# HumaticsLAB/SEAM-Match-RCNN

Hardware: NVIDIA B200
Metric: pair_scores_per_sec (higher is better)
Workload: dtype f32 (fp16-operand tcgen05 pass nominates candidates, every result re-scored in f32)

## Files before the change

seam-match-rcnn_b200/csrc/score_exact.cuh:

```cuda
#pragma once
#include <type_traits>
#include <climits>
#include <cstdint>
#include <cuda_fp16.h>
#include "exchange.cuh"
#include "fold.cuh"
#include "score_tc.cuh"
#include "sm100_ptx.cuh"
#include "warp_sort.cuh"

namespace seam {
namespace exact {

constexpr float FP16_MAX = 65504.f;
constexpr float EPS_COEFF = 9.9e-4f;
constexpr float TAG_REL_ERR = 8e-6f;

__device__ __forceinline__ float softmax1(float l0, float l1) {
  const float m = fmaxf(l0, l1);
  const float e0 = expf(l0 - m), e1 = expf(l1 - m);
  return e1 / (e0 + e1);
}

struct Slice {
  float4 lo, hi;
};
__device__ __forceinline__ Slice load_slice(const float* row, int lane) {
  Slice s;
  s.lo = *reinterpret_cast<const float4*>(row + 4 * lane);
  s.hi = *reinterpret_cast<const float4*>(row + 128 + 4 * lane);
  return s;
}
__device__ __forceinline__ float4 widen4(uint2 v) {
  const float2 a = __half22float2(*reinterpret_cast<const __half2*>(&v.x));
  const float2 b = __half22float2(*reinterpret_cast<const __half2*>(&v.y));
  return make_float4(a.x, a.y, b.x, b.y);
}
__device__ __forceinline__ Slice load_slice(const __half* row, int lane) {
  Slice s;
  s.lo = widen4(*reinterpret_cast<const uint2*>(row + 4 * lane));
  s.hi = widen4(*reinterpret_cast<const uint2*>(row + 128 + 4 * lane));
  return s;
}
typedef unsigned long long u64;
__device__ __forceinline__ u64 pk2(float lo, float hi) {
  u64 r;
  asm("mov.b64 %0, {%1, %2};" : "=l"(r) : "f"(lo), "f"(hi));
  return r;
}
__device__ __forceinline__ float sum2(u64 v) {
  float lo, hi;
  asm("mov.b64 {%0, %1}, %2;" : "=f"(lo), "=f"(hi) : "l"(v));
  return lo + hi;
}
__device__ __forceinline__ void sqdiff_dot2(const Slice& q, const Slice& g, const Slice& w0, const Slice& w1,
                                            float& p0, float& p1) {
  u64 a0, a1, d, s;
#define SEAM_TERM2(F, X, Y, FIRST)                                                                   \
  asm("sub.rn.f32x2 %0, %1, %2;" : "=l"(d) : "l"(pk2(q.F.X, q.F.Y)), "l"(pk2(g.F.X, g.F.Y)));      \
  asm("mul.rn.f32x2 %0, %1, %1;" : "=l"(s) : "l"(d));                                               \
  if (FIRST) {                                                                                       \
    asm("mul.rn.f32x2 %0, %1, %2;" : "=l"(a0) : "l"(pk2(w0.F.X, w0.F.Y)), "l"(s));                  \
    asm("mul.rn.f32x2 %0, %1, %2;" : "=l"(a1) : "l"(pk2(w1.F.X, w1.F.Y)), "l"(s));                  \
  } else {                                                                                           \
    asm("fma.rn.f32x2 %0, %1, %2, %0;" : "+l"(a0) : "l"(pk2(w0.F.X, w0.F.Y)), "l"(s));              \
    asm("fma.rn.f32x2 %0, %1, %2, %0;" : "+l"(a1) : "l"(pk2(w1.F.X, w1.F.Y)), "l"(s));              \
  }
  SEAM_TERM2(lo, x, y, true) SEAM_TERM2(lo, z, w, false) SEAM_TERM2(hi, x, y, false) SEAM_TERM2(hi, z, w, false)
#undef SEAM_TERM2
  p0 = sum2(a0);
  p1 = sum2(a1);
}
template <typename Row>
__device__ __forceinline__ void pair_logits(const Slice& q, const Row* grow, const Slice& w0, const Slice& w1,
                                            float b0, float b1, int lane, float& l0, float& l1) {
  const Slice g = load_slice(grow, lane);
  float p0, p1;
  sqdiff_dot2(q, g, w0, w1, p0, p1);
  l0 = ptx::warp_sum_b(p0) + b0;
  l1 = ptx::warp_sum_b(p1) + b1;
}

template <typename Row>
__global__ void __launch_bounds__(256) prep_gallery_kernel(const Row* __restrict__ g, int G,
                                                           const float* __restrict__ fold, __half* __restrict__ g16,
                                                           float* __restrict__ cg, float* __restrict__ gstat) {
  const int warp = threadIdx.x >> 5, lane = threadIdx.x & 31;
  const int j = blockIdx.x * 8 + warp;
  if (j >= G) return;
  const Slice x = load_slice(g + (size_t)j * 256, lane);
  const Slice dw = load_slice(fold + Fold::DW, lane);
  const float xs[8] = {x.lo.x, x.lo.y, x.lo.z, x.lo.w, x.hi.x, x.hi.y, x.hi.z, x.hi.w};
  const float ds[8] = {dw.lo.x, dw.lo.y, dw.lo.z, dw.lo.w, dw.hi.x, dw.hi.y, dw.hi.z, dw.hi.w};
  float c = 0.f, n2 = 0.f, amax = 0.f;
  __half h[8];
#pragma unroll
  for (int e = 0; e < 8; ++e) {
    c = fmaf(ds[e], xs[e] * xs[e], c);
    n2 = fmaf(xs[e], xs[e], n2);
    amax = fmaxf(amax, fabsf(xs[e]));
    h[e] = __float2half_rn(xs[e]);
  }
  if constexpr (std::is_same<Row, float>::value) {
    __half* dst = g16 + (size_t)j * 256;
    *reinterpret_cast<uint2*>(dst + 4 * lane) = *reinterpret_cast<const uint2*>(&h[0]);
    *reinterpret_cast<uint2*>(dst + 128 + 4 * lane) = *reinterpret_cast<const uint2*>(&h[4]);
  }
  c = ptx::warp_sum(c);
  n2 = ptx::warp_sum(n2);
  amax = ptx::warp_max(amax);
  if (lane == 0) {
    cg[j] = c;
    atomicMax(reinterpret_cast<unsigned int*>(gstat), __float_as_uint(sqrtf(n2)));
    if (!(amax < FP16_MAX)) atomicMax(reinterpret_cast<unsigned int*>(gstat + 1), __float_as_uint(1.f));
  }
}

__global__ void __launch_bounds__(256) prep_queries_kernel(const float* q, int Q,
                                                           const float* __restrict__ fold, __half* __restrict__ a16,
                                                           float* __restrict__ rq, float* __restrict__ anorm,
                                                           uint32_t* __restrict__ thr_global,
                                                           uint32_t* __restrict__ rowflag,
                                                           int32_t* __restrict__ counters,
                                                           int32_t* __restrict__ xdone, const int x_on,
                                                           const xchg::Exchange xc) {
  const int warp = threadIdx.x >> 5, lane = threadIdx.x & 31;
  const int i = blockIdx.x * 8 + warp;
  if (x_on) {
    const uint32_t step = xchg::current_step(xc);
    xchg::wait_all(xc, xchg::KIND_Q, step);
    q = xc.q_all[xc.rank] + (size_t)(step & 1u) * xc.Q * 256;
  }
  if (blockIdx.x == 0 && threadIdx.x == 0) {
    counters[0] = 0;
    counters[1] = 0;
  }
  if (i >= Q) return;
  const Slice x = load_slice(q + (size_t)i * 256, lane);
  const Slice dw = load_slice(fold + Fold::DW, lane);
  const float xs[8] = {x.lo.x, x.lo.y, x.lo.z, x.lo.w, x.hi.x, x.hi.y, x.hi.z, x.hi.w};
  const float ds[8] = {dw.lo.x, dw.lo.y, dw.lo.z, dw.lo.w, dw.hi.x, dw.hi.y, dw.hi.z, dw.hi.w};
  float r = 0.f, n2 = 0.f, amax = 0.f;
  __half h[8];
#pragma unroll
  for (int e = 0; e < 8; ++e) {
    const float a = -2.f * ds[e] * xs[e];
    r = fmaf(ds[e], xs[e] * xs[e], r);
    n2 = fmaf(a, a, n2);
    amax = fmaxf(amax, fabsf(a));
    h[e] = __float2half_rn(a);
  }
  __half* dst = a16 + (size_t)i * 256;
  *reinterpret_cast<uint2*>(dst + 4 * lane) = *reinterpret_cast<const uint2*>(&h[0]);
  *reinterpret_cast<uint2*>(dst + 128 + 4 * lane) = *reinterpret_cast<const uint2*>(&h[4]);
  r = ptx::warp_sum(r);
  n2 = ptx::warp_sum(n2);
  amax = ptx::warp_max(amax);
  if (lane == 0) {
    rq[i] = r;
    anorm[i] = sqrtf(n2);
    thr_global[i] = ptx::float_to_ordered(-INFINITY);
    rowflag[i] = 0;
    if (xdone) xdone[i] = 0;
    if (!(amax < FP16_MAX)) atomicExch(counters + 1, 1);
  }
}

struct RescoreParams {
  const float* q;
  const void* g;
  const float* fold;
  const uint2* rowbuf;
  const uint32_t* rowcnt;
  const uint32_t* rowflag;
  const uint32_t* thr_global;
  const float* gmax;
  const float* rq;
  const float* anorm;
  const float* gstat;
  int Q, G, nlists, CAP, k, index_offset;
  float* out_score;
  float* out_margin;
  int32_t* out_idx;
  int32_t* counters;
  int32_t* fallback_rows;
  int x_on;
  xchg::Exchange x;
  score::TilePlan plan;
};

struct TopkDest {
  float* score;
  float* margin;
  int32_t* idx;
};
__device__ __forceinline__ TopkDest topk_dest(int x_on, const xchg::Exchange& x, uint32_t step, int qi, int k,
                                              float* out_score, float* out_margin, int32_t* out_idx) {
  TopkDest d;
  if (!x_on) {
    const size_t o = (size_t)qi * k;
    d.score = out_score + o;
    d.margin = out_margin + o;
    d.idx = out_idx + o;
  } else {
    const int ow = xchg::owner_of(x, qi);
    const size_t o = ((((size_t)(step & 1u) * x.world + x.rank) * x.own_max) + (size_t)(qi - x.q_lo[ow])) * k;
    d.score = nullptr;
    d.margin = x.list_margin[ow] + o;
    d.idx = x.list_idx[ow] + o;
  }
  return d;
}

constexpr int RS_SUBL = 4;
constexpr int RESCORE_WBUF = 160;

__device__ __forceinline__ void rescore_merge32(const uint2* wb, int begin, int end, float& cv, uint32_t& cidx,
                                                int lane) {
  float v = -INFINITY;
  uint32_t id = 0xffffffffu;
  if (begin + lane < end) {
    const uint2 e = wb[begin + lane];
    v = __uint_as_float(e.x);
    id = e.y;
  }
  const float worst = __shfl_sync(ptx::FULL_MASK, cv, 31);
  if (!(v > worst)) {
    v = -INFINITY;
    id = 0xffffffffu;
  }
  if (!__any_sync(ptx::FULL_MASK, v > -INFINITY)) return;
  wsort::sort32<false>(v, id, lane);
  if (v > cv) {
    cv = v;
    cidx = id;
  }
  wsort::merge32<true>(cv, cidx, lane);
}

template <typename Row>
__global__ void __launch_bounds__(256) rescore_kernel(const RescoreParams p) {
  __shared__ uint2 wbuf[8][RESCORE_WBUF];
  __shared__ uint4 qbuf[8][64];
  __shared__ uint32_t qcol[8][64];
  const int warp = threadIdx.x >> 5, lane = threadIdx.x & 31;
  const int qi = blockIdx.x * 8 + warp;
  if (qi >= p.Q) return;
  const uint32_t xstep = p.x_on ? xchg::current_step(p.x) : 0u;
  const float* qbase = p.x_on ? p.x.q_all[p.x.rank] + (size_t)(xstep & 1u) * p.x.Q * 256 : p.q;
  const bool overflow = p.counters[1] != 0 || p.gstat[1] != 0.f;
  bool certified = !overflow && p.rowflag[qi] == 0;
  const float tau = ptx::ordered_to_float(p.thr_global[qi]);
  const int nl_valid = min(p.nlists, 4 * score::pieces_of_row(p.plan, qi));
  float cv = -INFINITY;
  uint32_t cidx = 0xffffffffu;
  uint2* wb = wbuf[warp];
  int fill = 0;
  float cut = tau;
  bool cut_strict = false;
  float cut_lo = tau > -INFINITY ? nextafterf(tau, -INFINITY) : -INFINITY;
  {
    const int nval = nl_valid * 16;
    const float* gmp = p.gmax + (size_t)qi * p.nlists * 16;
    auto start_cut = [&](auto nk_tag) {
      constexpr int NK = decltype(nk_tag)::value;
      uint32_t key[NK];
#pragma unroll
      for (int u = 0; u < NK; ++u) {
        const int i = lane + 32 * u;
        key[u] = i < nval ? ptx::float_to_ordered(gmp[i]) : 0u;
      }
      uint32_t lmax = key[0];
#pragma unroll
      for (int j = 1; j < NK; ++j) lmax = max(lmax, key[j]);
      const uint32_t hi = __reduce_max_sync(ptx::FULL_MASK, lmax);
      const uint32_t lo = __reduce_min_sync(ptx::FULL_MASK, lmax);
      uint32_t K = lo;
      if (hi != lo) {
        const int b0 = 31 - __clz(hi ^ lo);
        K = hi & ~((2u << b0) - 1u);
        for (int b = b0; b >= 0 && b > b0 - 8; --b) {
          const uint32_t T = K | (1u << b);
          uint32_t c = 0;
#pragma unroll
          for (int j = 0; j < NK; ++j)
            asm("{\n.reg .pred p;\nsetp.ge.u32 p, %1, %2;\n@p add.u32 %0, %0, 1;\n}\n" : "+r"(c) : "r"(key[j]), "r"(T));
          if (__reduce_add_sync(ptx::FULL_MASK, c) >= 32u) K = T;
        }
      }
      const float tt = ptx::ordered_to_float(K);
      if (K != 0 && tt > cut) {
        cut = tt;
        cut_lo = nextafterf(tt, -INFINITY);
      }
    };
    if (nval <= 128) start_cut(std::integral_constant<int, 4>{});
    else if (nval <= 256) start_cut(std::integral_constant<int, 8>{});
  }
  const int capq = p.CAP / 2;
  const uint4* rowq = reinterpret_cast<const uint4*>(p.rowbuf) + (size_t)qi * p.nlists * capq;
  uint4* qb = qbuf[warp];
  uint32_t* qc = qcol[warp];
  int qfill = 0;
  auto expand = [&](int start, int count) {
    uint4 rec = make_uint4(0u, 0u, 0u, 0u);
    uint32_t col = 0;
    const bool have = lane < count;
    if (have) {
      rec = qb[start + lane];
      col = qc[start + lane];
    }
    const uint32_t wv[4] = {rec.x, rec.y, rec.z, rec.w};
#pragma unroll
    for (int el = 0; el < 4; ++el) {
      const float ev = __uint_as_float(wv[el]);
      const bool pass = have && ev > cut_lo;
      const uint32_t mask = __ballot_sync(ptx::FULL_MASK, pass);
      if (mask == 0u) continue;
      if (pass) wb[fill + __popc(mask & ((1u << lane) - 1u))] = make_uint2(wv[el], col + el);
      fill += __popc(mask);
    }
    if (fill >= 32) {
      __syncwarp();
      while (fill >= 32) {
        rescore_merge32(wb, fill - 32, fill, cv, cidx, lane);
        fill -= 32;
      }
      const float worst = __shfl_sync(ptx::FULL_MASK, cv, 31);
      if (worst > cut || (worst == cut && worst > -INFINITY)) {
        cut = worst;
        cut_strict = true;
        cut_lo = worst;
      }
    }
    __syncwarp();
  };
  for (int l0 = 0; l0 < nl_valid && certified; l0 += 32) {
    const int my_l = l0 + lane;
    uint32_t my_n = my_l < nl_valid ? p.rowcnt[(size_t)qi * p.nlists + my_l] : 0u;
    if (__any_sync(ptx::FULL_MASK, my_n > (uint32_t)capq)) {
      certified = false;
      break;
    }
    const int nl = min(32, nl_valid - l0);
    for (int j0 = 0; j0 < nl; j0 += RS_SUBL) {
      int n4[RS_SUBL];
      int nmax = 0;
#pragma unroll
      for (int u = 0; u < RS_SUBL; ++u) {
        n4[u] = (int)__shfl_sync(ptx::FULL_MASK, my_n, j0 + u);
        nmax = max(nmax, n4[u]);
      }
      const uint4* lp = rowq + (size_t)(l0 + j0) * capq + lane;
      for (int base = 0; base < nmax; base += 32) {
        uint4 e[RS_SUBL];
#pragma unroll
        for (int u = 0; u < RS_SUBL; ++u)
          e[u] = base + lane < n4[u] ? __ldcs(lp + (size_t)u * capq + base)
                                     : make_uint4(0xff800000u, 0xff800000u, 0xff800000u, 0xff800000u);
#pragma unroll
        for (int u = 0; u < RS_SUBL; ++u) {
          const float m = fmaxf(fmaxf(__uint_as_float(e[u].x), __uint_as_float(e[u].y)),
                                fmaxf(__uint_as_float(e[u].z), __uint_as_float(e[u].w)));
          const bool pass = m > cut_lo;
          const uint32_t mask = __ballot_sync(ptx::FULL_MASK, pass);
          if (mask == 0u) continue;
          if (pass) {
            const int pos = qfill + __popc(mask & ((1u << lane) - 1u));
            qb[pos] = e[u];
            qc[pos] = score::quad_first_col(e[u], l0 + j0 + u);
          }
          qfill += __popc(mask);
          if (qfill >= 32) {
            __syncwarp();
            expand(qfill - 32, 32);
            qfill -= 32;
          }
        }
      }
    }
  }
  __syncwarp();
  if (certified && qfill > 0) expand(0, qfill);
  __syncwarp();
  if (certified && fill > 0) rescore_merge32(wb, 0, fill, cv, cidx, lane);
  const bool valid = (int)cidx >= 0;
  const int n_valid = __popc(__ballot_sync(ptx::FULL_MASK, valid));
  if (n_valid < min(32, p.G)) certified = false;
  const float a_k = __shfl_sync(ptx::FULL_MASK, cv, min(p.k, 32) - 1);
  const float amax = ptx::warp_max(valid ? fabsf(cv) : 0.f);
  const float eps = EPS_COEFF * p.anorm[qi] * p.gstat[0] + 1e-5f + TAG_REL_ERR * amax;
  const float cutoff = a_k - 2.f * eps;
  const bool in_S = valid && cv >= cutoff;
  const uint32_t smask = __ballot_sync(ptx::FULL_MASK, in_S);
  if (p.G > 32 && (smask >> 31)) certified = false;
  const int ns = __popc(smask);

  const Slice qs = load_slice(qbase + (size_t)qi * 256, lane);
  const Slice w0 = load_slice(p.fold + Fold::LAST_W, lane);
  const Slice w1 = load_slice(p.fold + Fold::LAST_W + 256, lane);
  const float b0 = p.fold[Fold::CONSTS + 5], b1 = p.fold[Fold::CONSTS + 6];
  float my_l0 = 0.f, my_l1 = 0.f;
  if (certified) {
    for (int c0 = 0; c0 < ns; c0 += 4) {
      Slice gs[4];
#pragma unroll
      for (int u = 0; u < 4; ++u) {
        const int idx = __shfl_sync(ptx::FULL_MASK, (int)cidx, min(c0 + u, ns - 1));
        gs[u] = load_slice(static_cast<const Row*>(p.g) + (size_t)idx * 256, lane);
      }
      float part[8];
#pragma unroll
      for (int u = 0; u < 4; ++u) sqdiff_dot2(qs, gs[u], w0, w1, part[2 * u], part[2 * u + 1]);
      const float tot = ptx::treduce<8>(part, lane);
      const int u_mine = lane - c0;
      const float l0 = __shfl_sync(ptx::FULL_MASK, tot, (2 * u_mine) & 7) + b0;
      const float l1 = __shfl_sync(ptx::FULL_MASK, tot, (2 * u_mine + 1) & 7) + b1;
      if (u_mine >= 0 && u_mine < 4) {
        my_l0 = l0;
        my_l1 = l1;
      }
    }
  }
  float d = in_S ? my_l1 - my_l0 : -INFINITY;
  int id = in_S ? (int)cidx : INT_MAX;
  const float approx_d = cv + p.rq[qi] + p.fold[Fold::CONSTS + 4];
  const bool violated = in_S && !(fabsf(d - approx_d) <= eps + 2e-5f * (1.f + fabsf(d)));
  if (__any_sync(ptx::FULL_MASK, violated)) certified = false;
  wsort::sort32_rank2(d, id, lane);
  if (lane < p.k) {
    const TopkDest dst = topk_dest(p.x_on, p.x, xstep, qi, p.k, p.out_score, p.out_margin, p.out_idx);
    const bool ok = id != INT_MAX;
    if (dst.score) dst.score[lane] = ok ? softmax1(0.f, d) : 0.f;
    dst.margin[lane] = d;
    dst.idx[lane] = ok ? id + p.index_offset : -1;
  }
  if (!certified && lane == 0) {
    const int slot = atomicAdd(p.counters, 1);
    p.fallback_rows[slot] = qi;
  }
}

struct ExactParams {
  const float* q;
  const void* g;
  const float* fold;
  int Q, G, k, index_offset;
  const int32_t* count;
  const int32_t* rows;
  float* out_score;
  float* out_margin;
  int32_t* out_idx;
  float* part_d;
  int32_t* part_i;
  int32_t* done;
  int x_on;
  xchg::Exchange x;
};

constexpr int EXACT_MIN_SLICE = 128;

template <typename Row>
__global__ void __launch_bounds__(256) exact_topk_kernel(const ExactParams p) {
  __shared__ float sd[8][32];
  __shared__ int si[8][32];
  __shared__ int s_last;
  const int warp = threadIdx.x >> 5, lane = threadIdx.x & 31;
  const int nrows = p.count ? *p.count : p.Q;
  const uint32_t xstep = p.x_on ? xchg::current_step(p.x) : 0u;
  const float* qbase = p.x_on ? p.x.q_all[p.x.rank] + (size_t)(xstep & 1u) * p.x.Q * 256 : p.q;
  int S = 1;
  if (p.part_d && nrows > 0 && nrows < (int)gridDim.x) S = max(1, min((int)gridDim.x / nrows, p.G / EXACT_MIN_SLICE));
  const long long units = (long long)nrows * S;
  if (units == 0) {
    if (p.x_on) xchg::signal_all(p.x, xchg::KIND_L, xstep, false);
    return;
  }
  const Slice w0 = load_slice(p.fold + Fold::LAST_W, lane);
  const Slice w1 = load_slice(p.fold + Fold::LAST_W + 256, lane);
  const float b0 = p.fold[Fold::CONSTS + 5], b1 = p.fold[Fold::CONSTS + 6];
  float cd;
  int cidx;
  auto cta_merge = [&]() {
    sd[warp][lane] = cd;
    si[warp][lane] = cidx;
    __syncthreads();
    if (warp == 0) {
      float dummy = 0.f;
      for (int w = 1; w < 8; ++w) {
        const float od = sd[w][31 - lane];
        const int oi = si[w][31 - lane];
        if (wsort::ranks_before(od, oi, cd, cidx)) {
          cd = od;
          cidx = oi;
        }
        wsort::merge32_rank(cd, cidx, dummy, lane);
      }
    }
  };
  auto write_row = [&](int qi) {
    if (lane < p.k) {
      const TopkDest dst = topk_dest(p.x_on, p.x, xstep, qi, p.k, p.out_score, p.out_margin, p.out_idx);
      const bool ok = cidx != INT_MAX;
      if (dst.score) dst.score[lane] = ok ? softmax1(0.f, cd) : 0.f;
      dst.margin[lane] = cd;
      dst.idx[lane] = ok ? cidx + p.index_offset : -1;
    }
  };
  for (long long e = blockIdx.x; e < units; e += gridDim.x) {
    const int r = (int)(e / S), sl = (int)(e - (long long)r * S);
    const int qi = p.count ? p.rows[r] : r;
    const int j_lo = (int)((long long)p.G * sl / S), j_hi = (int)((long long)p.G * (sl + 1) / S);
    const Slice qs = load_slice(qbase + (size_t)qi * 256, lane);
    cd = -INFINITY;
    cidx = INT_MAX;
    for (int j0 = j_lo + 4 * warp; j0 < j_hi; j0 += 32) {
      Slice gs[4];
#pragma unroll
      for (int u = 0; u < 4; ++u) gs[u] = load_slice(static_cast<const Row*>(p.g) + (size_t)min(j0 + u, j_hi - 1) * 256, lane);
      float part[8];
#pragma unroll
      for (int u = 0; u < 4; ++u) sqdiff_dot2(qs, gs[u], w0, w1, part[2 * u], part[2 * u + 1]);
      const float tot = ptx::treduce<8>(part, lane);
#pragma unroll
      for (int u = 0; u < 4; ++u) {
        const float l0 = __shfl_sync(ptx::FULL_MASK, tot, 2 * u) + b0;
        const float l1 = __shfl_sync(ptx::FULL_MASK, tot, 2 * u + 1) + b1;
        const float d = l1 - l0;
        const int j = j0 + u;
        const float wd = __shfl_sync(ptx::FULL_MASK, cd, 31);
        const int wi = __shfl_sync(ptx::FULL_MASK, cidx, 31);
        if (j < j_hi && wsort::ranks_before(d, j, wd, wi)) {
          const int pos = __popc(__ballot_sync(ptx::FULL_MASK, wsort::ranks_before(cd, cidx, d, j)));
          const float ud = __shfl_up_sync(ptx::FULL_MASK, cd, 1);
          const int ui = __shfl_up_sync(ptx::FULL_MASK, cidx, 1);
          if (lane > pos) {
            cd = ud;
            cidx = ui;
          } else if (lane == pos) {
            cd = d;
            cidx = j;
          }
        }
      }
    }
    cta_merge();
    if (S == 1) {
      if (warp == 0) write_row(qi);
      __syncthreads();
      continue;
    }
    if (warp == 0) {
      __stcg(p.part_d + (size_t)e * 32 + lane, cd);
      __stcg(p.part_i + (size_t)e * 32 + lane, cidx);
      __threadfence();
      __syncwarp();
      if (lane == 0) s_last = atomicAdd(p.done + r, 1) == S - 1;
    }
    __syncthreads();
    if (s_last) {
      __threadfence();
      cd = -INFINITY;
      cidx = INT_MAX;
      float dummy = 0.f;
      for (int s2 = warp; s2 < S; s2 += 8) {
        const size_t o = ((size_t)r * S + s2) * 32 + (31 - lane);
        const float od = __ldcg(p.part_d + o);
        const int oi = __ldcg(p.part_i + o);
        if (wsort::ranks_before(od, oi, cd, cidx)) {
          cd = od;
          cidx = oi;
        }
        wsort::merge32_rank(cd, cidx, dummy, lane);
      }
      __syncthreads();
      cta_merge();
      if (warp == 0) {
        write_row(qi);
        if (lane == 0) p.done[r] = 0;
      }
    }
    __syncthreads();
  }
  if (p.x_on) {
    __syncthreads();
    xchg::signal_all(p.x, xchg::KIND_L, xstep, (long long)blockIdx.x < units);
  }
}

template <bool PROB>
__global__ void __launch_bounds__(256) dense_logits_kernel(const float* __restrict__ q, int Q,
                                                           const float* __restrict__ g, int G,
                                                           const float* __restrict__ fold, float* __restrict__ x5) {
  __shared__ float qs[32][129];
  __shared__ float gs[32][129];
  __shared__ float ws[2][256];
  const int t = threadIdx.x;
  const int i0 = blockIdx.y * 32, j0 = blockIdx.x * 32;
  ws[0][t] = fold[Fold::LAST_W + t];
  ws[1][t] = fold[Fold::LAST_W + 256 + t];
  const int tx = t & 31, ty = t >> 5;
  float l0[4] = {}, l1[4] = {};
  for (int kh = 0; kh < 256; kh += 128) {
    __syncthreads();
    for (int e = t; e < 32 * 128; e += 256) {
      const int r = e >> 7, c = e & 127;
      qs[r][c] = (i0 + r < Q) ? q[(size_t)(i0 + r) * 256 + kh + c] : 0.f;
      gs[r][c] = (j0 + r < G) ? g[(size_t)(j0 + r) * 256 + kh + c] : 0.f;
    }
    __syncthreads();
    for (int k = 0; k < 128; ++k) {
      const float gv = gs[tx][k];
      const float wa = ws[0][kh + k], wb = ws[1][kh + k];
#pragma unroll
      for (int u = 0; u < 4; ++u) {
        const float d = qs[ty * 4 + u][k] - gv;
        const float s = d * d;
        l0[u] = fmaf(wa, s, l0[u]);
        l1[u] = fmaf(wb, s, l1[u]);
      }
    }
  }
  const float b0 = fold[Fold::CONSTS + 5], b1 = fold[Fold::CONSTS + 6];
#pragma unroll
  for (int u = 0; u < 4; ++u) {
    const int i = i0 + ty * 4 + u, j = j0 + tx;
    if (i < Q && j < G) {
      if constexpr (PROB) {
        x5[(size_t)i * G + j] = softmax1(l0[u] + b0, l1[u] + b1);
      } else {
        float2 o = make_float2(l0[u] + b0, l1[u] + b1);
        *reinterpret_cast<float2*>(x5 + ((size_t)i * G + j) * 2) = o;
      }
    }
  }
}

struct FusedDistParams {
  const float* frames;
  const int32_t* start;
  const float* g;
  const int32_t* target;
  const float* fold;
  int P, G;
  int32_t* rank_avg;
  int32_t* rank_max;
};
constexpr int FD_ROWS = 1024, FD_FRAMES = 16;

__global__ void __launch_bounds__(256) fused_dist_rank_kernel(const FusedDistParams p) {
  __shared__ __align__(16) float fs[FD_FRAMES][256];
  __shared__ float acc_sum[FD_ROWS + 1], acc_max[FD_ROWS + 1];
  __shared__ int cnt_s[2];
  const int warp = threadIdx.x >> 5, lane = threadIdx.x & 31;
  const int prod = blockIdx.x, j0 = blockIdx.y * FD_ROWS;
  const int f0 = p.start[prod], nf = p.start[prod + 1] - f0;
  if (nf <= 0) {
    if (blockIdx.y == 0 && threadIdx.x == 0) {
      p.rank_avg[prod] = p.G;
      p.rank_max[prod] = p.G;
    }
    return;
  }
  const int rows = min(FD_ROWS, p.G - j0);
  const int tj = p.target[prod];
  for (int i = threadIdx.x; i <= FD_ROWS; i += 256) {
    acc_sum[i] = 0.f;
    acc_max[i] = -INFINITY;
  }
  if (threadIdx.x < 2) cnt_s[threadIdx.x] = 0;
  const Slice w0 = load_slice(p.fold + Fold::LAST_W, lane);
  const Slice w1 = load_slice(p.fold + Fold::LAST_W + 256, lane);
  const float b0 = p.fold[Fold::CONSTS + 5], b1 = p.fold[Fold::CONSTS + 6];
  for (int c0 = 0; c0 < nf; c0 += FD_FRAMES) {
    const int nc = min(FD_FRAMES, nf - c0);
    __syncthreads();
    for (int e = threadIdx.x; e < nc * 64; e += 256)
      reinterpret_cast<float4*>(&fs[0][0])[e] = reinterpret_cast<const float4*>(p.frames + (size_t)(f0 + c0) * 256)[e];
    __syncthreads();
    for (int r = warp; r <= rows; r += 8) {
      const int j = r < rows ? j0 + r : tj;
      const int slot = r < rows ? r : FD_ROWS;
      const Slice gs = load_slice(p.g + (size_t)j * 256, lane);
      float sum = 0.f, mx = -INFINITY;
      for (int fb = 0; fb < nc; fb += 4) {
        float part[8];
#pragma unroll
        for (int u = 0; u < 4; ++u) {
          const Slice fr = load_slice(&fs[min(fb + u, nc - 1)][0], lane);
          sqdiff_dot2(fr, gs, w0, w1, part[2 * u], part[2 * u + 1]);
        }
        const float tot = ptx::treduce<8>(part, lane);
#pragma unroll
        for (int u = 0; u < 4; ++u) {
          const float l0 = __shfl_sync(ptx::FULL_MASK, tot, 2 * u) + b0;
          const float l1 = __shfl_sync(ptx::FULL_MASK, tot, 2 * u + 1) + b1;
          if (fb + u < nc) {
            const float pr = softmax1(l0, l1);
            sum += pr;
            mx = fmaxf(mx, pr);
          }
        }
      }
      if (lane == 0) {
        acc_sum[slot] += sum;
        acc_max[slot] = fmaxf(acc_max[slot], mx);
      }
    }
  }
  __syncthreads();
  const float inv = 1.f / (float)nf;
  const float tavg = acc_sum[FD_ROWS] * inv, tmax = acc_max[FD_ROWS];
  int ca = 0, cm = 0;
  for (int i = threadIdx.x; i < rows; i += 256) {
    const int j = j0 + i;
    const float a = acc_sum[i] * inv, m = acc_max[i];
    ca += (a > tavg || (a == tavg && j < tj)) ? 1 : 0;
    cm += (m > tmax || (m == tmax && j < tj)) ? 1 : 0;
  }
  ca = __reduce_add_sync(ptx::FULL_MASK, ca);
  cm = __reduce_add_sync(ptx::FULL_MASK, cm);
  if (lane == 0) {
    atomicAdd(&cnt_s[0], ca);
    atomicAdd(&cnt_s[1], cm);
  }
  __syncthreads();
  if (threadIdx.x == 0) {
    atomicAdd(p.rank_avg + prod, cnt_s[0]);
    atomicAdd(p.rank_max + prod, cnt_s[1]);
  }
}

template <typename Row>
__global__ void __launch_bounds__(256) rank_of_target_kernel(const float* __restrict__ q, int Q,
                                                             const Row* __restrict__ g, int G,
                                                             const int32_t* __restrict__ target,
                                                             const float* __restrict__ fold,
                                                             const int32_t* __restrict__ count,
                                                             const int32_t* __restrict__ rows,
                                                             int32_t* __restrict__ out_rank,
                                                             float* __restrict__ out_margin) {
  __shared__ int cnt_s[8];
  const int warp = threadIdx.x >> 5, lane = threadIdx.x & 31;
  const Slice w0 = load_slice(fold + Fold::LAST_W, lane);
  const Slice w1 = load_slice(fold + Fold::LAST_W + 256, lane);
  const float b0 = fold[Fold::CONSTS + 5], b1 = fold[Fold::CONSTS + 6];
  const int nrows = count ? *count : Q;
  for (int e = blockIdx.x; e < nrows; e += gridDim.x) {
    const int qi = count ? rows[e] : e;
    const Slice qs = load_slice(q + (size_t)qi * 256, lane);
    const int tj = target[qi];
    float l0, l1;
    pair_logits(qs, g + (size_t)tj * 256, w0, w1, b0, b1, lane, l0, l1);
    const float dt = l1 - l0;
    int cnt = 0;
    for (int j = warp; j < G; j += 8) {
      pair_logits(qs, g + (size_t)j * 256, w0, w1, b0, b1, lane, l0, l1);
      if (wsort::ranks_before(l1 - l0, j, dt, tj)) ++cnt;
    }
    if (lane == 0) cnt_s[warp] = cnt;
    __syncthreads();
    if (threadIdx.x == 0) {
      int tot = 0;
      for (int w = 0; w < 8; ++w) tot += cnt_s[w];
      out_rank[qi] = tot;
      if (out_margin) out_margin[qi] = dt;
    }
    __syncthreads();
  }
}

template <typename Row>
__global__ void __launch_bounds__(256) rank_prep_kernel(const float* __restrict__ q, int Q, const Row* __restrict__ g,
                                                        const int32_t* __restrict__ target,
                                                        const float* __restrict__ fold, const float* __restrict__ rq,
                                                        const float* __restrict__ anorm,
                                                        const float* __restrict__ gstat, float* __restrict__ lo,
                                                        float* __restrict__ hi, float* __restrict__ dtarget,
                                                        int32_t* __restrict__ above, int nlists) {
  const int warp = threadIdx.x >> 5, lane = threadIdx.x & 31;
  const int qi = blockIdx.x * 8 + warp;
  if (qi >= Q) return;
  const Slice w0 = load_slice(fold + Fold::LAST_W, lane);
  const Slice w1 = load_slice(fold + Fold::LAST_W + 256, lane);
  const float b0 = fold[Fold::CONSTS + 5], b1 = fold[Fold::CONSTS + 6];
  const Slice qs = load_slice(q + (size_t)qi * 256, lane);
  float l0, l1;
  pair_logits(qs, g + (size_t)target[qi] * 256, w0, w1, b0, b1, lane, l0, l1);
  const float dt = l1 - l0;
  for (int l = lane; l < nlists; l += 32) above[(size_t)qi * nlists + l] = 0;
  if (lane == 0) {
    const float vstar = dt - rq[qi] - fold[Fold::CONSTS + 4];
    const float e0 = EPS_COEFF * anorm[qi] * gstat[0] + 1e-5f;
    const float E = e0 + TAG_REL_ERR * (fabsf(vstar) + e0) + 4e-6f * (1.f + fabsf(dt) + fabsf(vstar));
    lo[qi] = vstar - E;
    hi[qi] = vstar + E;
    dtarget[qi] = dt;
  }
}

struct RankResolveParams {
  const float* q;
  const void* g;
  const float* fold;
  const uint2* rowbuf;
  const uint32_t* rowcnt;
  const uint32_t* rowflag;
  const int32_t* above;
  const float* lo;
  const float* hi;
  const float* dtarget;
  const float* rq;
  const float* gstat;
  const int32_t* target;
  int Q, G, nlists, CAP;
  score::TilePlan plan;
  int32_t* out_rank;
  float* out_margin;
  int32_t* counters;
  int32_t* fallback_rows;
};
constexpr int RANK_CAND = 96;

template <typename Row>
__global__ void __launch_bounds__(256) rank_resolve_kernel(const RankResolveParams p) {
  __shared__ uint2 cand[8][RANK_CAND + 128];
  const int warp = threadIdx.x >> 5, lane = threadIdx.x & 31;
  const int qi = blockIdx.x * 8 + warp;
  if (qi >= p.Q) return;
  const bool overflow = p.counters[1] != 0 || p.gstat[1] != 0.f;
  bool ok = !overflow && p.rowflag[qi] == 0;
  const float lo = p.lo[qi], hi = p.hi[qi], dt = p.dtarget[qi];
  const int tj = p.target[qi];
  const int capq = p.CAP / 2;
  const uint4* rowq = reinterpret_cast<const uint4*>(p.rowbuf) + (size_t)qi * p.nlists * capq;
  uint2* cb = cand[warp];
  const Slice qs = load_slice(p.q + (size_t)qi * 256, lane);
  const Slice w0 = load_slice(p.fold + Fold::LAST_W, lane);
  const Slice w1 = load_slice(p.fold + Fold::LAST_W + 256, lane);
  const float b0 = p.fold[Fold::CONSTS + 5], b1 = p.fold[Fold::CONSTS + 6];
  const float eps = 0.5f * (hi - lo);
  const float shift = p.rq[qi] + p.fold[Fold::CONSTS + 4];
  int total = 0, fill = 0, exact_before = 0;
  auto decide = [&]() {
    __syncwarp();
    for (int c0 = 0; c0 < fill; c0 += 4) {
      Slice gs[4];
      uint2 ce[4];
#pragma unroll
      for (int u = 0; u < 4; ++u) {
        ce[u] = cb[min(c0 + u, fill - 1)];
        gs[u] = load_slice(static_cast<const Row*>(p.g) + (size_t)ce[u].y * 256, lane);
      }
      float part[8];
#pragma unroll
      for (int u = 0; u < 4; ++u) sqdiff_dot2(qs, gs[u], w0, w1, part[2 * u], part[2 * u + 1]);
      const float tot = ptx::treduce<8>(part, lane);
#pragma unroll
      for (int u = 0; u < 4; ++u) {
        const float l0v = __shfl_sync(ptx::FULL_MASK, tot, 2 * u) + b0;
        const float l1v = __shfl_sync(ptx::FULL_MASK, tot, 2 * u + 1) + b1;
        const float d = l1v - l0v;
        if (c0 + u < fill) {
          if (wsort::ranks_before(d, (int)ce[u].y, dt, tj)) ++exact_before;
          if (!(fabsf(d - (__uint_as_float(ce[u].x) + shift)) <= eps)) ok = false;
        }
      }
    }
    fill = 0;
    __syncwarp();
  };
  const int nl_valid = min(p.nlists, 4 * score::pieces_of_row(p.plan, qi));
  for (int l0 = 0; l0 < nl_valid && ok; l0 += 32) {
    const int my_l = l0 + lane;
    const uint32_t my_n = my_l < nl_valid ? p.rowcnt[(size_t)qi * p.nlists + my_l] : 0u;
    total += my_l < nl_valid ? p.above[(size_t)qi * p.nlists + my_l] : 0;
    if (__any_sync(ptx::FULL_MASK, my_n > (uint32_t)capq)) ok = false;
    const int nl = min(32, nl_valid - l0);
    for (int j = 0; j < nl && ok; ++j) {
      const int n = (int)__shfl_sync(ptx::FULL_MASK, my_n, j);
      const uint4* lp = rowq + (size_t)(l0 + j) * capq;
      for (int base = 0; base < n && ok; base += 32) {
        const bool have = base + lane < n;
        const uint4 rec = have ? __ldcs(lp + base + lane) : make_uint4(0u, 0u, 0u, 0u);
        const uint32_t wv[4] = {rec.x, rec.y, rec.z, rec.w};
        const uint32_t col = score::quad_first_col(rec, l0 + j);
#pragma unroll
        for (int el = 0; el < 4; ++el) {
          const float ev = __uint_as_float(wv[el]);
          const bool in_band = have && ev > lo && !(ev > hi);
          const uint32_t mask = __ballot_sync(ptx::FULL_MASK, in_band);
          if (mask == 0u) continue;
          if (in_band) cb[fill + __popc(mask & ((1u << lane) - 1u))] = make_uint2(wv[el], col + el);
          fill += __popc(mask);
        }
        if (fill >= RANK_CAND) decide();
      }
    }
  }
  total = __reduce_add_sync(ptx::FULL_MASK, total);
  if (ok && fill > 0) decide();
  if (lane == 0) {
    if (ok) {
      p.out_rank[qi] = total + exact_before;
      if (p.out_margin) p.out_margin[qi] = dt;
    } else {
      const int slot = atomicAdd(p.counters, 1);
      p.fallback_rows[slot] = qi;
    }
  }
}

__global__ void __launch_bounds__(256) merge_topk_kernel(const float* __restrict__ scores,
                                                         const float* __restrict__ margins,
                                                         const int32_t* __restrict__ idx, int N, int Q, int k,
                                                         float* __restrict__ out_score,
                                                         float* __restrict__ out_margin,
                                                         int32_t* __restrict__ out_idx) {
  const int warp = threadIdx.x >> 5, lane = threadIdx.x & 31;
  const int qi = blockIdx.x * 8 + warp;
  if (qi >= Q) return;
  float d = -INFINITY, s = 0.f;
  int id = INT_MAX;
  for (int n = 0; n < N; ++n) {
    const size_t base = ((size_t)n * Q + qi) * k;
    if (n == 0) {
      if (lane < k && idx[base + lane] >= 0) {
        d = margins[base + lane];
        s = scores ? scores[base + lane] : 0.f;
        id = idx[base + lane];
      }
    } else {
      const int e = 31 - lane;
      float od = -INFINITY, os = 0.f;
      int oi = INT_MAX;
      if (e < k && idx[base + e] >= 0) {
        od = margins[base + e];
        os = scores ? scores[base + e] : 0.f;
        oi = idx[base + e];
      }
      if (wsort::ranks_before(od, oi, d, id)) {
        d = od;
        id = oi;
        s = os;
      }
      wsort::merge32_rank(d, id, s, lane);
    }
  }
  if (lane < k) {
    const size_t o = (size_t)qi * k + lane;
    const bool ok = id != INT_MAX;
    out_score[o] = ok ? (scores ? s : softmax1(0.f, d)) : 0.f;
    out_margin[o] = ok ? d : -INFINITY;
    out_idx[o] = ok ? id : -1;
  }
}

__global__ void __launch_bounds__(256) merge_sharded_kernel(const xchg::Exchange x, float* __restrict__ out_score,
                                                            float* __restrict__ out_margin,
                                                            int32_t* __restrict__ out_idx) {
  const int warp = threadIdx.x >> 5, lane = threadIdx.x & 31;
  const uint32_t step = xchg::current_step(x);
  xchg::wait_all(x, xchg::KIND_L, step);
  const int own = x.q_lo[x.rank + 1] - x.q_lo[x.rank], k = x.k;
  const int qo = blockIdx.x * 8 + warp;
  if (qo < own) {
    const float* margins = x.list_margin[x.rank] + (size_t)(step & 1u) * x.world * x.own_max * k;
    const int32_t* idx = x.list_idx[x.rank] + (size_t)(step & 1u) * x.world * x.own_max * k;
    float d = -INFINITY, s = 0.f;
    int id = INT_MAX;
    for (int n = 0; n < x.world; ++n) {
      const size_t base = ((size_t)n * x.own_max + qo) * k;
      const int e = n == 0 ? lane : 31 - lane;
      float od = -INFINITY;
      int oi = INT_MAX;
      if (e < k) {
        const int32_t ii = __ldcg(idx + base + e);
        if (ii >= 0) {
          od = __ldcg(margins + base + e);
          oi = ii;
        }
      }
      if (n == 0) {
        d = od;
        id = oi;
      } else {
        if (wsort::ranks_before(od, oi, d, id)) {
          d = od;
          id = oi;
        }
        wsort::merge32_rank(d, id, s, lane);
      }
    }
    if (lane < k) {
      const bool ok = id != INT_MAX;
      const float sc = ok ? softmax1(0.f, d) : 0.f;
      const float dm = ok ? d : -INFINITY;
      const int ii = ok ? id : -1;
      if (x.final_score[0]) {
        const size_t o = (size_t)(x.q_lo[x.rank] + qo) * k + lane;
        if (x.final_score_mc) {
          x.final_score_mc[o] = sc;
          x.final_margin_mc[o] = dm;
          x.final_idx_mc[o] = ii;
        } else {
          for (int r = 0; r < x.world; ++r) {
            x.final_score[r][o] = sc;
            x.final_margin[r][o] = dm;
            x.final_idx[r][o] = ii;
          }
        }
      } else {
        const size_t o = (size_t)qo * k + lane;
        out_score[o] = sc;
        out_margin[o] = dm;
        out_idx[o] = ii;
      }
    }
  }
  __syncthreads();
  if (xchg::signal_all(x, xchg::KIND_F, step)) {
    if (x.final_score[0]) {
      for (int r = 0; r < x.world; ++r) {
        const uint32_t* f = x.flags[x.rank] + xchg::KIND_F * xchg::MAX_WORLD + r;
        uint64_t t0 = 0;
        while ((int32_t)(xchg::ld_acquire_sys(f) - step) < 0) {
          __nanosleep(100);
          const uint64_t now = ptx::globaltimer_ns();
          if (t0 == 0) t0 = now;
          else if (now - t0 > 10000000000ull) ptx::watchdog_trap(210u, (uint32_t)r, step);
        }
      }
    }
    *reinterpret_cast<volatile uint32_t*>(x.step) = step + 1u;
  }
}

}
}
```

seam-match-rcnn_b200/csrc/warp_sort.cuh:

```cuda
#pragma once
#include <cstdint>
#include "sm100_ptx.cuh"

namespace seam {
namespace wsort {

template <bool DESC>
__device__ __forceinline__ void cmpx(float& v, uint32_t& p, int lane, int j, int k) {
  const float ov = __shfl_xor_sync(ptx::FULL_MASK, v, j);
  const uint32_t op = __shfl_xor_sync(ptx::FULL_MASK, p, j);
  const bool keep_min = ((((lane & k) == 0) == ((lane & j) == 0)) != DESC);
  const float nv = keep_min ? fminf(v, ov) : fmaxf(v, ov);
  if (nv != v) p = op;
  v = nv;
}
template <bool DESC>
__device__ __forceinline__ void sort32(float& v, uint32_t& p, int lane) {
#pragma unroll
  for (int k = 2; k <= 32; k <<= 1)
#pragma unroll
    for (int j = k >> 1; j > 0; j >>= 1) cmpx<DESC>(v, p, lane, j, k);
}
template <bool DESC>
__device__ __forceinline__ void merge32(float& v, uint32_t& p, int lane) {
#pragma unroll
  for (int j = 16; j > 0; j >>= 1) cmpx<DESC>(v, p, lane, j, 32);
}

__device__ __forceinline__ bool ranks_before(float da, int ia, float db, int ib) {
  return da > db || (da == db && ia < ib);
}
__device__ __forceinline__ void cmpx_rank(float& d, int& i, float& s, int lane, int j, int k) {
  const float od = __shfl_xor_sync(ptx::FULL_MASK, d, j);
  const int oi = __shfl_xor_sync(ptx::FULL_MASK, i, j);
  const float os = __shfl_xor_sync(ptx::FULL_MASK, s, j);
  const bool up = (lane & k) == 0;
  const bool lower = (lane & j) == 0;
  const bool keep_better = (lower == up);
  const bool take = keep_better ? ranks_before(od, oi, d, i) : ranks_before(d, i, od, oi);
  if (take) {
    d = od;
    i = oi;
    s = os;
  }
}
__device__ __forceinline__ void cmpx_rank2(float& d, int& i, int lane, int j, int k) {
  const float od = __shfl_xor_sync(ptx::FULL_MASK, d, j);
  const int oi = __shfl_xor_sync(ptx::FULL_MASK, i, j);
  const bool up = (lane & k) == 0;
  const bool lower = (lane & j) == 0;
  const bool keep_better = (lower == up);
  const bool take = keep_better ? ranks_before(od, oi, d, i) : ranks_before(d, i, od, oi);
  if (take) {
    d = od;
    i = oi;
  }
}
__device__ __forceinline__ void sort32_rank2(float& d, int& i, int lane) {
  uint32_t hi = ptx::float_to_ordered(d), lo = ~(uint32_t)i;
#pragma unroll
  for (int k = 2; k <= 32; k <<= 1)
#pragma unroll
    for (int j = k >> 1; j > 0; j >>= 1) {
      const uint32_t ohi = __shfl_xor_sync(ptx::FULL_MASK, hi, j);
      const uint32_t olo = __shfl_xor_sync(ptx::FULL_MASK, lo, j);
      const bool keep_better = ((lane & k) == 0) == ((lane & j) == 0);
      const bool other_better = ohi > hi || (ohi == hi && olo > lo);
      if (other_better == keep_better) {
        hi = ohi;
        lo = olo;
      }
    }
  d = ptx::ordered_to_float(hi);
  i = (int)~lo;
}
__device__ __forceinline__ void sort32_rank(float& d, int& i, float& s, int lane) {
#pragma unroll
  for (int k = 2; k <= 32; k <<= 1)
#pragma unroll
    for (int j = k >> 1; j > 0; j >>= 1) cmpx_rank(d, i, s, lane, j, k);
}
__device__ __forceinline__ void merge32_rank(float& d, int& i, float& s, int lane) {
#pragma unroll
  for (int j = 16; j > 0; j >>= 1) cmpx_rank(d, i, s, lane, j, 32);
}

}
}
```

Baseline: 1023 billion.

## Replace bitonic merge top-32 in rescore with buffered radix-bisect selection

The rescore kernel no longer keeps a running top-32 through repeated bitonic sort/merge networks on shuffles. Passing candidates are appended to a larger per-warp shared buffer, which is compacted by a bisection threshold search once it fills. The final k-th value, minimum and maximum come from counting ranks, and output order comes from a shared-memory rank count instead of a bitonic sort. It also exits early to the fallback path, defers the query pointer setup, and adds a min-blocks launch bound. The intent is to cut shuffle-heavy sorting work per query row, at the cost of extra shared-memory passes and more intricate tie handling.

New measurement: 1036 billion (median of 6 runs). 1.01x the previous value.

```diff
diff --git a/seam-match-rcnn_b200/csrc/score_exact.cuh b/seam-match-rcnn_b200/csrc/score_exact.cuh
--- a/seam-match-rcnn_b200/csrc/score_exact.cuh
+++ b/seam-match-rcnn_b200/csrc/score_exact.cuh
@@ -213,51 +213,48 @@
 }
 
 constexpr int RS_SUBL = 4;
-constexpr int RESCORE_WBUF = 160;
-
-__device__ __forceinline__ void rescore_merge32(const uint2* wb, int begin, int end, float& cv, uint32_t& cidx,
-                                                int lane) {
-  float v = -INFINITY;
-  uint32_t id = 0xffffffffu;
-  if (begin + lane < end) {
-    const uint2 e = wb[begin + lane];
-    v = __uint_as_float(e.x);
-    id = e.y;
-  }
-  const float worst = __shfl_sync(ptx::FULL_MASK, cv, 31);
-  if (!(v > worst)) {
-    v = -INFINITY;
-    id = 0xffffffffu;
-  }
-  if (!__any_sync(ptx::FULL_MASK, v > -INFINITY)) return;
-  wsort::sort32<false>(v, id, lane);
-  if (v > cv) {
-    cv = v;
-    cidx = id;
-  }
-  wsort::merge32<true>(cv, cidx, lane);
+constexpr int RS_EBUF = 192;
+constexpr int RS_SELECT = 64;
+
+__device__ __forceinline__ void add_if_ge(uint32_t& c, uint32_t key, uint32_t T) {
+  asm("{\n.reg .pred p;\nsetp.ge.u32 p, %1, %2;\n@p add.u32 %0, %0, 1;\n}\n" : "+r"(c) : "r"(key), "r"(T));
+}
+
+template <typename CountGe>
+__device__ __forceinline__ uint32_t bisect_desc(uint32_t lo, uint32_t hi, uint32_t r, int nbits, CountGe count_ge) {
+  if (hi == lo) return lo;
+  const int b0 = 31 - __clz(hi ^ lo);
+  uint32_t K = hi & ~((2u << b0) - 1u);
+  for (int b = b0; b >= 0 && b > b0 - nbits; --b) {
+    const uint32_t T = K | (1u << b);
+    if (__reduce_add_sync(ptx::FULL_MASK, count_ge(T)) >= r) K = T;
+  }
+  return K;
 }
 
 template <typename Row>
-__global__ void __launch_bounds__(256) rescore_kernel(const RescoreParams p) {
-  __shared__ uint2 wbuf[8][RESCORE_WBUF];
+__global__ void __launch_bounds__(256, 4) rescore_kernel(const RescoreParams p) {
+  __shared__ __align__(16) uint2 ebuf[8][RS_EBUF];
   __shared__ uint4 qbuf[8][64];
   __shared__ uint32_t qcol[8][64];
   const int warp = threadIdx.x >> 5, lane = threadIdx.x & 31;
   const int qi = blockIdx.x * 8 + warp;
   if (qi >= p.Q) return;
-  const uint32_t xstep = p.x_on ? xchg::current_step(p.x) : 0u;
-  const float* qbase = p.x_on ? p.x.q_all[p.x.rank] + (size_t)(xstep & 1u) * p.x.Q * 256 : p.q;
+  const uint32_t lt_mask = (1u << lane) - 1u;
+  auto fall_back = [&]() {
+    if (lane == 0) {
+      const int slot = atomicAdd(p.counters, 1);
+      p.fallback_rows[slot] = qi;
+    }
+  };
   const bool overflow = p.counters[1] != 0 || p.gstat[1] != 0.f;
-  bool certified = !overflow && p.rowflag[qi] == 0;
+  if (overflow || p.rowflag[qi] != 0) {
+    fall_back();
+    return;
+  }
+  bool certified = true;
   const float tau = ptx::ordered_to_float(p.thr_global[qi]);
   const int nl_valid = min(p.nlists, 4 * score::pieces_of_row(p.plan, qi));
-  float cv = -INFINITY;
-  uint32_t cidx = 0xffffffffu;
-  uint2* wb = wbuf[warp];
-  int fill = 0;
-  float cut = tau;
-  bool cut_strict = false;
   float cut_lo = tau > -INFINITY ? nextafterf(tau, -INFINITY) : -INFINITY;
   {
     const int nval = nl_valid * 16;
@@ -275,30 +272,57 @@
       for (int j = 1; j < NK; ++j) lmax = max(lmax, key[j]);
       const uint32_t hi = __reduce_max_sync(ptx::FULL_MASK, lmax);
       const uint32_t lo = __reduce_min_sync(ptx::FULL_MASK, lmax);
-      uint32_t K = lo;
-      if (hi != lo) {
-        const int b0 = 31 - __clz(hi ^ lo);
-        K = hi & ~((2u << b0) - 1u);
-        for (int b = b0; b >= 0 && b > b0 - 8; --b) {
-          const uint32_t T = K | (1u << b);
-          uint32_t c = 0;
-#pragma unroll
-          for (int j = 0; j < NK; ++j)
-            asm("{\n.reg .pred p;\nsetp.ge.u32 p, %1, %2;\n@p add.u32 %0, %0, 1;\n}\n" : "+r"(c) : "r"(key[j]), "r"(T));
-          if (__reduce_add_sync(ptx::FULL_MASK, c) >= 32u) K = T;
-        }
-      }
+      const uint32_t K = bisect_desc(lo, hi, 32u, 8, [&](uint32_t T) {
+        uint32_t c = 0;
+#pragma unroll
+        for (int j = 0; j < NK; ++j) add_if_ge(c, key[j], T);
+        return c;
+      });
       const float tt = ptx::ordered_to_float(K);
-      if (K != 0 && tt > cut) {
-        cut = tt;
-        cut_lo = nextafterf(tt, -INFINITY);
-      }
+      if (K != 0 && tt > tau) cut_lo = nextafterf(tt, -INFINITY);
     };
     if (nval <= 128) start_cut(std::integral_constant<int, 4>{});
     else if (nval <= 256) start_cut(std::integral_constant<int, 8>{});
   }
   const int capq = p.CAP / 2;
   const uint4* rowq = reinterpret_cast<const uint4*>(p.rowbuf) + (size_t)qi * p.nlists * capq;
+  uint2* eb = ebuf[warp];
+  int fill = 0;
+  auto compact = [&]() {
+    __syncwarp();
+    uint32_t lo = 0xffffffffu, hi = 0u;
+    for (int i = lane; i < fill; i += 32) {
+      const uint32_t key = ptx::float_to_ordered(__uint_as_float(eb[i].x));
+      lo = min(lo, key);
+      hi = max(hi, key);
+    }
+    lo = __reduce_min_sync(ptx::FULL_MASK, lo);
+    hi = __reduce_max_sync(ptx::FULL_MASK, hi);
+    const uint32_t T = bisect_desc(lo, hi, 32u, 32, [&](uint32_t t) {
+      uint32_t c = 0;
+      for (int i = lane; i < fill; i += 32) add_if_ge(c, ptx::float_to_ordered(__uint_as_float(eb[i].x)), t);
+      return c;
+    });
+    uint32_t above = 0;
+    for (int i = lane; i < fill; i += 32) above += ptx::float_to_ordered(__uint_as_float(eb[i].x)) > T;
+    const int room = 32 - (int)__reduce_add_sync(ptx::FULL_MASK, above);
+    int kept = 0, ties = 0;
+    for (int i0 = 0; i0 < fill; i0 += 32) {
+      const int i = i0 + lane;
+      const uint2 e = i < fill ? eb[i] : make_uint2(0u, 0u);
+      const uint32_t key = ptx::float_to_ordered(__uint_as_float(e.x));
+      const bool tie = i < fill && key == T;
+      const uint32_t tm = __ballot_sync(ptx::FULL_MASK, tie);
+      const bool keep = (i < fill && key > T) || (tie && ties + __popc(tm & lt_mask) < room);
+      ties += __popc(tm);
+      const uint32_t km = __ballot_sync(ptx::FULL_MASK, keep);
+      if (keep) eb[kept + __popc(km & lt_mask)] = e;
+      kept += __popc(km);
+    }
+    fill = kept;
+    cut_lo = ptx::ordered_to_float(T);
+    __syncwarp();
+  };
   uint4* qb = qbuf[warp];
   uint32_t* qc = qcol[warp];
   int qfill = 0;
@@ -310,34 +334,20 @@
       rec = qb[start + lane];
       col = qc[start + lane];
     }
+    if (fill > RS_EBUF - 128) compact();
     const uint32_t wv[4] = {rec.x, rec.y, rec.z, rec.w};
 #pragma unroll
     for (int el = 0; el < 4; ++el) {
-      const float ev = __uint_as_float(wv[el]);
-      const bool pass = have && ev > cut_lo;
-      const uint32_t mask = __ballot_sync(ptx::FULL_MASK, pass);
-      if (mask == 0u) continue;
-      if (pass) wb[fill + __popc(mask & ((1u << lane) - 1u))] = make_uint2(wv[el], col + el);
+      const bool keep = have && __uint_as_float(wv[el]) > cut_lo;
+      const uint32_t mask = __ballot_sync(ptx::FULL_MASK, keep);
+      if (keep) eb[fill + __popc(mask & lt_mask)] = make_uint2(wv[el], col + el);
       fill += __popc(mask);
-    }
-    if (fill >= 32) {
-      __syncwarp();
-      while (fill >= 32) {
-        rescore_merge32(wb, fill - 32, fill, cv, cidx, lane);
-        fill -= 32;
-      }
-      const float worst = __shfl_sync(ptx::FULL_MASK, cv, 31);
-      if (worst > cut || (worst == cut && worst > -INFINITY)) {
-        cut = worst;
-        cut_strict = true;
-        cut_lo = worst;
-      }
     }
     __syncwarp();
   };
   for (int l0 = 0; l0 < nl_valid && certified; l0 += 32) {
     const int my_l = l0 + lane;
-    uint32_t my_n = my_l < nl_valid ? p.rowcnt[(size_t)qi * p.nlists + my_l] : 0u;
+    const uint32_t my_n = my_l < nl_valid ? p.rowcnt[(size_t)qi * p.nlists + my_l] : 0u;
     if (__any_sync(ptx::FULL_MASK, my_n > (uint32_t)capq)) {
       certified = false;
       break;
@@ -366,7 +376,7 @@
           const uint32_t mask = __ballot_sync(ptx::FULL_MASK, pass);
           if (mask == 0u) continue;
           if (pass) {
-            const int pos = qfill + __popc(mask & ((1u << lane) - 1u));
+            const int pos = qfill + __popc(mask & lt_mask);
             qb[pos] = e[u];
             qc[pos] = score::quad_first_col(e[u], l0 + j0 + u);
           }
@@ -383,61 +393,122 @@
   __syncwarp();
   if (certified && qfill > 0) expand(0, qfill);
   __syncwarp();
-  if (certified && fill > 0) rescore_merge32(wb, 0, fill, cv, cidx, lane);
-  const bool valid = (int)cidx >= 0;
-  const int n_valid = __popc(__ballot_sync(ptx::FULL_MASK, valid));
-  if (n_valid < min(32, p.G)) certified = false;
-  const float a_k = __shfl_sync(ptx::FULL_MASK, cv, min(p.k, 32) - 1);
-  const float amax = ptx::warp_max(valid ? fabsf(cv) : 0.f);
+  if (certified && fill > RS_SELECT) compact();
+  const int n = fill;
+  if (!certified || n < min(32, p.G)) {
+    fall_back();
+    return;
+  }
+  uint32_t* kb32 = reinterpret_cast<uint32_t*>(eb + RS_SELECT);
+  uint32_t key[2], above[2] = {0u, 0u};
+#pragma unroll
+  for (int u = 0; u < 2; ++u) {
+    const int i = lane + 32 * u;
+    key[u] = i < n ? ptx::float_to_ordered(__uint_as_float(eb[i].x)) : 0u;
+    kb32[i] = key[u];
+  }
+  __syncwarp();
+  for (int j = 0; j < n; j += 4) {
+    const uint4 o = *reinterpret_cast<const uint4*>(kb32 + j);
+#pragma unroll
+    for (int u = 0; u < 2; ++u) {
+      const uint32_t T = key[u] + 1u;
+      add_if_ge(above[u], o.x, T);
+      add_if_ge(above[u], o.y, T);
+      add_if_ge(above[u], o.z, T);
+      add_if_ge(above[u], o.w, T);
+    }
+  }
+  auto kth = [&](uint32_t r) {
+    uint32_t m = 0xffffffffu;
+#pragma unroll
+    for (int u = 0; u < 2; ++u)
+      if (lane + 32 * u < n && above[u] < r) m = min(m, key[u]);
+    return __reduce_min_sync(ptx::FULL_MASK, m);
+  };
+  const uint32_t kmin = kth(32u);
+  const uint32_t hi = kth(1u);
+  const int kk = min(p.k, 32);
+  const float a_k = n < kk ? -INFINITY : ptx::ordered_to_float(kth((uint32_t)kk));
+  const float vmin = ptx::ordered_to_float(kmin);
+  const float amax = fmaxf(fabsf(ptx::ordered_to_float(hi)), fabsf(vmin));
   const float eps = EPS_COEFF * p.anorm[qi] * p.gstat[0] + 1e-5f + TAG_REL_ERR * amax;
   const float cutoff = a_k - 2.f * eps;
-  const bool in_S = valid && cv >= cutoff;
-  const uint32_t smask = __ballot_sync(ptx::FULL_MASK, in_S);
-  if (p.G > 32 && (smask >> 31)) certified = false;
-  const int ns = __popc(smask);
-
+  if (p.G > 32 && n >= 32 && vmin >= cutoff) {
+    fall_back();
+    return;
+  }
+  int ns = 0;
+#pragma unroll
+  for (int u = 0; u < 2; ++u) {
+    const int i = lane + 32 * u;
+    const bool in = i < n && ptx::ordered_to_float(key[u]) >= cutoff;
+    const uint2 e = in ? eb[i] : make_uint2(0u, 0u);
+    const uint32_t mask = __ballot_sync(ptx::FULL_MASK, in);
+    if (in) eb[ns + __popc(mask & lt_mask)] = e;
+    ns += __popc(mask);
+  }
+  __syncwarp();
+  const bool in_S = lane < ns;
+  float cv = 0.f;
+  int cidx = 0;
+  if (in_S) {
+    const uint2 e = eb[lane];
+    cv = __uint_as_float(e.x);
+    cidx = (int)e.y;
+  }
+
+  const uint32_t xstep = p.x_on ? xchg::current_step(p.x) : 0u;
+  const float* qbase = p.x_on ? p.x.q_all[p.x.rank] + (size_t)(xstep & 1u) * p.x.Q * 256 : p.q;
   const Slice qs = load_slice(qbase + (size_t)qi * 256, lane);
   const Slice w0 = load_slice(p.fold + Fold::LAST_W, lane);
   const Slice w1 = load_slice(p.fold + Fold::LAST_W + 256, lane);
   const float b0 = p.fold[Fold::CONSTS + 5], b1 = p.fold[Fold::CONSTS + 6];
   float my_l0 = 0.f, my_l1 = 0.f;
-  if (certified) {
-    for (int c0 = 0; c0 < ns; c0 += 4) {
-      Slice gs[4];
-#pragma unroll
-      for (int u = 0; u < 4; ++u) {
-        const int idx = __shfl_sync(ptx::FULL_MASK, (int)cidx, min(c0 + u, ns - 1));
-        gs[u] = load_slice(static_cast<const Row*>(p.g) + (size_t)idx * 256, lane);
-      }
-      float part[8];
-#pragma unroll
-      for (int u = 0; u < 4; ++u) sqdiff_dot2(qs, gs[u], w0, w1, part[2 * u], part[2 * u + 1]);
-      const float tot = ptx::treduce<8>(part, lane);
-      const int u_mine = lane - c0;
-      const float l0 = __shfl_sync(ptx::FULL_MASK, tot, (2 * u_mine) & 7) + b0;
-      const float l1 = __shfl_sync(ptx::FULL_MASK, tot, (2 * u_mine + 1) & 7) + b1;
-      if (u_mine >= 0 && u_mine < 4) {
-        my_l0 = l0;
-        my_l1 = l1;
-      }
-    }
-  }
-  float d = in_S ? my_l1 - my_l0 : -INFINITY;
-  int id = in_S ? (int)cidx : INT_MAX;
+  for (int c0 = 0; c0 < ns; c0 += 4) {
+    Slice gs[4];
+#pragma unroll
+    for (int u = 0; u < 4; ++u) {
+      const int idx = __shfl_sync(ptx::FULL_MASK, cidx, min(c0 + u, ns - 1));
+      gs[u] = load_slice(static_cast<const Row*>(p.g) + (size_t)idx * 256, lane);
+    }
+    float part[8];
+#pragma unroll
+    for (int u = 0; u < 4; ++u) sqdiff_dot2(qs, gs[u], w0, w1, part[2 * u], part[2 * u + 1]);
+    const float tot = ptx::treduce<8>(part, lane);
+    const int u_mine = lane - c0;
+    const float l0 = __shfl_sync(ptx::FULL_MASK, tot, (2 * u_mine) & 7) + b0;
+    const float l1 = __shfl_sync(ptx::FULL_MASK, tot, (2 * u_mine + 1) & 7) + b1;
+    if (u_mine >= 0 && u_mine < 4) {
+      my_l0 = l0;
+      my_l1 = l1;
+    }
+  }
+  const float d = my_l1 - my_l0;
   const float approx_d = cv + p.rq[qi] + p.fold[Fold::CONSTS + 4];
   const bool violated = in_S && !(fabsf(d - approx_d) <= eps + 2e-5f * (1.f + fabsf(d)));
-  if (__any_sync(ptx::FULL_MASK, violated)) certified = false;
-  wsort::sort32_rank2(d, id, lane);
-  if (lane < p.k) {
-    const TopkDest dst = topk_dest(p.x_on, p.x, xstep, qi, p.k, p.out_score, p.out_margin, p.out_idx);
-    const bool ok = id != INT_MAX;
-    if (dst.score) dst.score[lane] = ok ? softmax1(0.f, d) : 0.f;
-    dst.margin[lane] = d;
-    dst.idx[lane] = ok ? id + p.index_offset : -1;
-  }
-  if (!certified && lane == 0) {
-    const int slot = atomicAdd(p.counters, 1);
-    p.fallback_rows[slot] = qi;
+  if (__any_sync(ptx::FULL_MASK, violated)) {
+    fall_back();
+    return;
+  }
+  const u64 rk = ((u64)ptx::float_to_ordered(d) << 32) | (uint32_t)~cidx;
+  u64* kb = reinterpret_cast<u64*>(eb);
+  __syncwarp();
+  if (in_S) kb[lane] = rk;
+  __syncwarp();
+  int rank = 0;
+  for (int j = 0; j < ns; ++j) rank += kb[j] > rk ? 1 : 0;
+  const TopkDest dst = topk_dest(p.x_on, p.x, xstep, qi, p.k, p.out_score, p.out_margin, p.out_idx);
+  if (in_S) {
+    if (rank < p.k) {
+      if (dst.score) dst.score[rank] = softmax1(0.f, d);
+      dst.margin[rank] = d;
+      dst.idx[rank] = cidx + p.index_offset;
+    }
+  } else if (lane < p.k) {
+    if (dst.score) dst.score[lane] = 0.f;
+    dst.margin[lane] = -INFINITY;
+    dst.idx[lane] = -1;
   }
 }
 
diff --git a/seam-match-rcnn_b200/csrc/warp_sort.cuh b/seam-match-rcnn_b200/csrc/warp_sort.cuh
--- a/seam-match-rcnn_b200/csrc/warp_sort.cuh
+++ b/seam-match-rcnn_b200/csrc/warp_sort.cuh
@@ -4,28 +4,6 @@
 
 namespace seam {
 namespace wsort {
-
-template <bool DESC>
-__device__ __forceinline__ void cmpx(float& v, uint32_t& p, int lane, int j, int k) {
-  const float ov = __shfl_xor_sync(ptx::FULL_MASK, v, j);
-  const uint32_t op = __shfl_xor_sync(ptx::FULL_MASK, p, j);
-  const bool keep_min = ((((lane & k) == 0) == ((lane & j) == 0)) != DESC);
-  const float nv = keep_min ? fminf(v, ov) : fmaxf(v, ov);
-  if (nv != v) p = op;
-  v = nv;
-}
-template <bool DESC>
-__device__ __forceinline__ void sort32(float& v, uint32_t& p, int lane) {
-#pragma unroll
-  for (int k = 2; k <= 32; k <<= 1)
-#pragma unroll
-    for (int j = k >> 1; j > 0; j >>= 1) cmpx<DESC>(v, p, lane, j, k);
-}
-template <bool DESC>
-__device__ __forceinline__ void merge32(float& v, uint32_t& p, int lane) {
-#pragma unroll
-  for (int j = 16; j > 0; j >>= 1) cmpx<DESC>(v, p, lane, j, 32);
-}
 
 __device__ __forceinline__ bool ranks_before(float da, int ia, float db, int ib) {
   return da > db || (da == db && ia < ib);
@@ -56,24 +34,6 @@
     i = oi;
   }
 }
-__device__ __forceinline__ void sort32_rank2(float& d, int& i, int lane) {
-  uint32_t hi = ptx::float_to_ordered(d), lo = ~(uint32_t)i;
-#pragma unroll
-  for (int k = 2; k <= 32; k <<= 1)
-#pragma unroll
-    for (int j = k >> 1; j > 0; j >>= 1) {
-      const uint32_t ohi = __shfl_xor_sync(ptx::FULL_MASK, hi, j);
-      const uint32_t olo = __shfl_xor_sync(ptx::FULL_MASK, lo, j);
-      const bool keep_better = ((lane & k) == 0) == ((lane & j) == 0);
-      const bool other_better = ohi > hi || (ohi == hi && olo > lo);
-      if (other_better == keep_better) {
-        hi = ohi;
-        lo = olo;
-      }
-    }
-  d = ptx::ordered_to_float(hi);
-  i = (int)~lo;
-}
 __device__ __forceinline__ void sort32_rank(float& d, int& i, float& s, int lane) {
 #pragma unroll
   for (int k = 2; k <= 32; k <<= 1)
```
